# OpenSLAM-org/openslam_g2o

Hardware: AMD Instinct MI355X
Metric: linear-solve ms/iter (buildSystem + setLambda + solve + restoreDiagonal), 100k-pose BA (lower is better)
Workload: dtype f64; 1 GPU; synthetic BA (BASELINE.json configs[3]): 100000 poses / 1000000 landmarks / 5000000 observations, BlockSolver_6_3 semantics, Schur + multifrontal block Cholesky, lambda=10; poses=100000, landmarks=1000000, edges=5000000, parallelism=1 GPU, edge_data=estimates+measurements in HBM, errors/Jacobians evaluated inside buildSystem, information=identity, declared for the whole edge set (not read per edge)

## Files before the change

### openslam_g2o_amd/csrc/block_solver.hip

```cpp
#include "block_solver.h"

#include <algorithm>
#include <atomic>
#include <chrono>
#include <cmath>
#include <cstring>
#include <numeric>

namespace g2ohip {

namespace {

constexpr int kThreads = 256;
constexpr int kMaxBlocks = 1024;

template <int CTRL>
__device__ __forceinline__ double dpp_permute(double v) {
  const int lo = __double2loint(v), hi = __double2hiint(v);
  const int lo2 = __builtin_amdgcn_update_dpp(lo, lo, CTRL, 0xf, 0xf, true);
  const int hi2 = __builtin_amdgcn_update_dpp(hi, hi, CTRL, 0xf, 0xf, true);
  return __hiloint2double(hi2, lo2);
}
template <int G>
__device__ __forceinline__ double group_sum(double v) {
  if (G >= 2) v += dpp_permute<0xB1>(v);
  if (G >= 4) v += dpp_permute<0x4E>(v);
  if (G >= 8) v += dpp_permute<0x141>(v);
  if (G >= 16) v += dpp_permute<0x140>(v);
  return v;
}

typedef double dbl2_u __attribute__((ext_vector_type(2), aligned(8)));
template <int N>
__device__ __forceinline__ void load_vec(const double* __restrict__ p, double (&v)[N]) {
#pragma unroll
  for (int i = 0; i + 1 < N; i += 2) {
    const dbl2_u t = *reinterpret_cast<const dbl2_u*>(p + i);
    v[i] = t.x;
    v[i + 1] = t.y;
  }
  if (N & 1) v[N - 1] = p[N - 1];
}
template <int N>
__device__ __forceinline__ void store_vec(double* __restrict__ p, const double (&v)[N]) {
#pragma unroll
  for (int i = 0; i + 1 < N; i += 2) {
    dbl2_u t;
    t.x = v[i];
    t.y = v[i + 1];
    *reinterpret_cast<dbl2_u*>(p + i) = t;
  }
  if (N & 1) p[N - 1] = v[N - 1];
}
typedef double dbl2_a __attribute__((ext_vector_type(2), aligned(16)));
template <int N>
__device__ __forceinline__ void lds_block(const double* p, double (&v)[N]) {
  if (N % 2 == 0) {
#pragma unroll
    for (int i = 0; i < N; i += 2) {
      const dbl2_a t = *reinterpret_cast<const dbl2_a*>(p + i);
      v[i] = t.x;
      v[i + 1] = t.y;
    }
  } else {
#pragma unroll
    for (int i = 0; i < N; ++i) v[i] = p[i];
  }
}
__device__ __forceinline__ int xcd_swizzle(int b, int nblocks) {
  const int per = nblocks >> 3;
  return (b < (per << 3)) ? (b & 7) * per + (b >> 3) : b;
}

__device__ __forceinline__ double robust_weight(int kind, double delta, double e2) {
  const double dsqr = delta * delta;
  switch (kind) {
    case 1: return (e2 <= dsqr) ? 1.0 : delta / sqrt(e2);
    case 2: return 1.0 / sqrt(e2 / dsqr + 1.0);
    case 3: return 1.0 / (e2 / dsqr + 1.0);
    case 4: return (e2 <= dsqr) ? 1.0 : 0.0;
    case 5: {
      double sc = (2.0 * delta) / (delta + e2);
      if (sc >= 1.0) sc = 1.0;
      return sc * sc;
    }
    default: return 1.0;
  }
}
__device__ __forceinline__ double robust_rho(int kind, double delta, double e2) {
  const double dsqr = delta * delta;
  switch (kind) {
    case 1: return (e2 <= dsqr) ? e2 : 2.0 * sqrt(e2) * delta - dsqr;
    case 2: return 2.0 * dsqr * (sqrt(e2 / dsqr + 1.0) - 1.0);
    case 3: return dsqr * log(e2 / dsqr + 1.0);
    case 4: return (e2 <= dsqr) ? e2 : dsqr;
    case 5: {
      double sc = (2.0 * delta) / (delta + e2);
      if (sc >= 1.0) sc = 1.0;
      return sc * e2 * sc;
    }
    default: return e2;
  }
}

template <bool CLS>
__device__ __forceinline__ int ba_edge_class(int camword, const double* __restrict__ ctab, double& f, double& cx, double& cy, int& kind,
                                             double& delta) {
  if constexpr (CLS) {
    const double* t = ctab + 5 * (size_t)((unsigned)camword >> 24);
    f = t[0]; cx = t[1]; cy = t[2]; kind = (int)t[3]; delta = t[4];
    return camword & 0xffffff;
  } else {
    return camword;
  }
}

template <int D, int DV, int G>
__global__ void __launch_bounds__(kThreads) assemble_vertex_kernel(int nV, const int* __restrict__ vptr, const int* __restrict__ vent,
                                       const double* __restrict__ J0, const double* __restrict__ J1,
                                       const double* __restrict__ omega, const double* __restrict__ err, int kind, double delta,
                                       double* __restrict__ H, const int* __restrict__ diag_blk, double* __restrict__ b,
                                       int accumulate, const double* __restrict__ rk) {
  const int gt = blockIdx.x * blockDim.x + threadIdx.x;
  const int v = gt / G, g = gt % G;
  const bool active = v < nV;
  double Hacc[DV * DV];
  double bacc[DV];
#pragma unroll
  for (int i = 0; i < DV * DV; ++i) Hacc[i] = 0.0;
#pragma unroll
  for (int i = 0; i < DV; ++i) bacc[i] = 0.0;
  const int k0 = active ? vptr[v] : 0, k1 = active ? vptr[v + 1] : 0;
  for (int k = k0 + g; k < k1; k += G) {
    const int ent = vent[k];
    const size_t e = (size_t)(ent >> 1);
    const double* Jp = ((ent & 1) ? J1 : J0) + e * (D * DV);
    const double* Op = omega + e * (D * D);
    const double* rp = err + e * D;
    double J[D * DV], O[D * D], r[D], Or[D];
    load_vec<D * DV>(Jp, J);
    load_vec<D * D>(Op, O);
    load_vec<D>(rp, r);
    double e2 = 0.0;
#pragma unroll
    for (int i = 0; i < D; ++i) {
      double t = 0.0;
#pragma unroll
      for (int j = 0; j < D; ++j) t += O[i + D * j] * r[j];
      Or[i] = t;
      e2 += r[i] * t;
    }
    const double w = rk ? robust_weight((int)rk[2 * e], rk[2 * e + 1], e2) : robust_weight(kind, delta, e2);
#pragma unroll
    for (int c = 0; c < DV; ++c) {
      double t = 0.0;
#pragma unroll
      for (int i = 0; i < D; ++i) t += J[i + D * c] * Or[i];
      bacc[c] -= w * t;
    }
#pragma unroll
    for (int c = 0; c < DV; ++c) {
      double OJ[D];
#pragma unroll
      for (int i = 0; i < D; ++i) {
        double t = 0.0;
#pragma unroll
        for (int j = 0; j < D; ++j) t += O[i + D * j] * J[j + D * c];
        OJ[i] = w * t;
      }
#pragma unroll
      for (int a = 0; a < DV; ++a) {
        double t = 0.0;
#pragma unroll
        for (int i = 0; i < D; ++i) t += J[i + D * a] * OJ[i];
        Hacc[a + DV * c] += t;
      }
    }
  }
  if (G > 1) {
#pragma unroll
    for (int i = 0; i < DV * DV; ++i) Hacc[i] = group_sum<G>(Hacc[i]);
#pragma unroll
// ... 882 lines not shown

__device__ __forceinline__ void ba_lm_accumulate(const BaEdgeLin& L, double (&H)[9], double (&b)[3], double (&OA)[6]) {
  const double w = L.w;
  const double O00 = w * L.O[0], O10 = w * L.O[1], O01 = w * L.O[2], O11 = w * L.O[3];
#pragma unroll
  for (int c = 0; c < 3; ++c) {
    OA[0 + 2 * c] = O00 * L.A[0 + 2 * c] + O01 * L.A[1 + 2 * c];
    OA[1 + 2 * c] = O10 * L.A[0 + 2 * c] + O11 * L.A[1 + 2 * c];
  }
  const double Or0 = O00 * L.r[0] + O01 * L.r[1], Or1 = O10 * L.r[0] + O11 * L.r[1];
#pragma unroll
  for (int c = 0; c < 3; ++c) {
    b[c] -= L.A[0 + 2 * c] * Or0 + L.A[1 + 2 * c] * Or1;
#pragma unroll
    for (int a = 0; a < 3; ++a) H[a + 3 * c] += L.A[0 + 2 * a] * OA[0 + 2 * c] + L.A[1 + 2 * a] * OA[1 + 2 * c];
  }
}
__device__ __forceinline__ void ba_hpl_block(const BaEdgeLin& L, const double (&OA)[6], double (&blk)[18]) {
#pragma unroll
  for (int c = 0; c < 3; ++c)
#pragma unroll
    for (int a = 0; a < 6; ++a) blk[a + 6 * c] = L.B[0 + 2 * a] * OA[0 + 2 * c] + L.B[1 + 2 * a] * OA[1 + 2 * c];
}

#ifndef G2OHIP_ASMLM_OCC
#define G2OHIP_ASMLM_OCC 4
#endif
template <int G, bool CLS = false>
__global__ void __launch_bounds__(kThreads, G2OHIP_ASMLM_OCC) ba_assemble_landmarks_kernel(
    int nL, const int* __restrict__ vptr, const int* __restrict__ vent, const double* __restrict__ cams, const double* __restrict__ pts,
    const int* __restrict__ cam_lm, const int* __restrict__ pt_lm, const double* __restrict__ meas_lm, const double* __restrict__ omega_lm,
    const int* __restrict__ hpl_lm, double f, double cx, double cy, int kind, double delta, double* __restrict__ Hll,
    double* __restrict__ bl, double* __restrict__ Hpl, double* __restrict__ err, int ident, const int* __restrict__ pl_colptr,
    int write_hpl, const double* __restrict__ ctab) {
  __shared__ __attribute__((aligned(16))) double stage[kThreads / 64][64 * 18];
  const int gt = blockIdx.x * blockDim.x + threadIdx.x;
  const int lm = gt / G, g = gt % G;
  const bool active = lm < nL;
  const int wave = threadIdx.x / 64, lane = threadIdx.x % 64;
  const int lm_w0 = min((gt - lane) / G, nL), lm_w1 = min(lm_w0 + 64 / G, nL);
  const int q_base = pl_colptr[lm_w0], nslots = pl_colptr[lm_w1] - q_base;
  const bool staged = nslots <= 64;
  double H[9], b[3];
#pragma unroll
  for (int i = 0; i < 9; ++i) H[i] = 0.0;
  b[0] = b[1] = b[2] = 0.0;
  const int k0 = active ? vptr[lm] : 0, k1 = active ? vptr[lm + 1] : 0;
  for (int k = k0 + g; k < k1; k += G) {
    const int e = vent[k] >> 1;
    double T[12], X[3], z2[2], Op[4];
    const double* Xp = pts + (size_t)pt_lm[k] * 3;
    X[0] = Xp[0]; X[1] = Xp[1]; X[2] = Xp[2];
    load_vec<12>(cams + (size_t)ba_edge_class<CLS>(cam_lm[k], ctab, f, cx, cy, kind, delta) * 12, T);
    load_vec<2>(meas_lm + (size_t)k * 2, z2);
    if (ident) {
      Op[0] = Op[3] = 1.0;
      Op[1] = Op[2] = 0.0;
    } else {
      load_vec<4>(omega_lm + (size_t)k * 4, Op);
    }
    BaEdgeLin L;
    ba_edge_linearize(T, X, z2, Op, f, cx, cy, kind, delta, true, L);
    store_vec<2>(err + (size_t)e * 2, L.r);
    double OA[6];
    ba_lm_accumulate(L, H, b, OA);
    const int q = write_hpl ? hpl_lm[k] : -1;
    if (q >= 0) {
      double blk[18];
      ba_hpl_block(L, OA, blk);
      if (staged) store_vec<18>(&stage[wave][(q - q_base) * 18], blk);
      else store_vec<18>(Hpl + (size_t)q * 18, blk);
    }
  }
  if (staged && write_hpl) {
    __builtin_amdgcn_wave_barrier();
    const dbl2_u* src = reinterpret_cast<const dbl2_u*>(&stage[wave][0]);
    dbl2_u* dst = reinterpret_cast<dbl2_u*>(Hpl + (size_t)q_base * 18);
    for (int t = lane; t < nslots * 9; t += 64) dst[t] = src[t];
  }
  if (G > 1) {
#pragma unroll
    for (int i = 0; i < 9; ++i) H[i] = group_sum<G>(H[i]);
#pragma unroll
    for (int i = 0; i < 3; ++i) b[i] = group_sum<G>(b[i]);
  }
  if (!active) return;
#pragma unroll
  for (int i = 0; i < 9; ++i)
    if (G == 1 || (i % G) == g) Hll[(size_t)lm * 9 + i] = H[i];
#pragma unroll
  for (int i = 0; i < 3; ++i)
    if (G == 1 || (i % G) == g) bl[(size_t)lm * 3 + i] = b[i];
}

template <int G, bool FLL, bool CLS = false>
__global__ void __launch_bounds__(kThreads, G2OHIP_SCHUR_OCC) ba_schur_tile_kernel(
    const int* __restrict__ tile_lm0, const double* __restrict__ cams, const double* __restrict__ pts, const int* __restrict__ cam_q,
    const int* __restrict__ pt_q, const double* __restrict__ meas_q, const double* __restrict__ omega_q, double f, double cx, double cy,
    int kind, double delta, int ident, double* __restrict__ Dinv, double* bl, const int* __restrict__ td_diag,
    const int* __restrict__ td_ptr, const int* __restrict__ te_pack, const unsigned short* __restrict__ te_lm, double* __restrict__ Pd,
    double* __restrict__ Pr, double* Hll, const double* __restrict__ lam, const int4* __restrict__ ll_rec,
    const int4* __restrict__ tile_ll, const int* __restrict__ ll_edge, double* __restrict__ err, const int2* __restrict__ tile_q2,
    int store_hll, const unsigned short* __restrict__ slot_lm, const double* __restrict__ ctab) {
  extern __shared__ __attribute__((aligned(16))) double smem[];
  constexpr int PD = 6, LD = 3, PL = PD * LD;
  const int t = xcd_swizzle(blockIdx.x, gridDim.x);
  const int* tm = tile_lm0 + (size_t)t * 8;
  const int l0 = tm[0], l1 = tm[1], q0 = tm[2], nslots = tm[3], nlm = l1 - l0;
  const int td0 = tm[4], td1 = tm[5], e0 = tm[6], ne = tm[7];
  const int2 t2 = FLL ? make_int2(0, 0) : tile_q2[t];
  const int ntot = nslots + t2.y;
  double* Bs = smem;
  double* Ds = Bs + ((ntot * PL + 1) & ~1);
  double* bsm = Ds + ((nlm * LD * LD + 1) & ~1);
  double* Cs = bsm + ((nlm * LD + 1) & ~1);
  int* ep = reinterpret_cast<int*>(Cs + nlm * TileSplit<LD>::CP);
  int* dptr = ep + ne;
  int* ddiag = dptr + (td1 - td0 + 1);
  int* neg_flag = ddiag + (td1 - td0);
  unsigned short* el = reinterpret_cast<unsigned short*>(neg_flag + kThreads / 64);
  const int tid = threadIdx.x, NT = blockDim.x;
  if ((tid & 63) == 0) neg_flag[tid >> 6] = 0;
  const int slot_lm_first = FLL ? 0 : (int)slot_lm[q0 + min(tid, nslots - 1)];
  {
    const double* srcD = Hll + (size_t)l0 * LD * LD;
    const double* srcb = bl + (size_t)l0 * LD;
    const int nD = nlm * LD * LD, nb = nlm * LD, ndp = td1 - td0 + 1;
    constexpr int UD = 3, UE = 4;
    double vD[UD], vb;
    int vE[UE], vP, vG;
    unsigned short vL[UE];
    const int s0 = min(tid, nslots - 1);
    int cq = 0, pq = 0;
    if constexpr (!FLL) {
      cq = cam_q[q0 + s0];
      pq = pt_q[q0 + s0];
#pragma unroll
      for (int u = 0; u < UD; ++u) vD[u] = srcD[min(tid + u * NT, nD - 1)];
      vb = srcb[min(tid, nb - 1)];
    }
    auto request_lists = [&]() {
#pragma unroll
      for (int u = 0; u < UE; ++u) {
        const int i = min(tid + u * NT, ne - 1);
        vE[u] = te_pack[e0 + i];
        vL[u] = te_lm[e0 + i];
      }
      vP = td_ptr[td0 + min(tid, ndp - 1)];
      vG = td_diag[td0 + min(tid, max(ndp - 2, 0))];
    };
    request_lists();
    if constexpr (FLL) {
      const int4 tl = tile_ll[t];
      for (int sb = 0; sb < tl.y; sb += NT) {
        const int si = sb + tid;
        const size_t sg = (size_t)tl.x + min(si, tl.y - 1);
        int4 rc = ll_rec[sg];
        if (si >= tl.y) rc.x = (int)0x80000fffu;
        const int ent = rc.x;
        const int krel = ent & 0xfff, K = (ent >> 12) & 0xff, lmi = (ent >> 20) & 0x7ff;
        const bool has = krel != 0xfff, head = ent >= 0;
        const int pos = head ? 0 : lmi;
        double v[9];
        double Bk[12], OAk[6];
#pragma unroll
        for (int i = 0; i < 12; ++i) Bk[i] = 0.0;
#pragma unroll
        for (int i = 0; i < 6; ++i) OAk[i] = 0.0;
#pragma unroll
        for (int i = 0; i < 9; ++i) v[i] = 0.0;
        {
          const int ci = ba_edge_class<CLS>(rc.y, ctab, f, cx, cy, kind, delta), pi = rc.z, q = rc.w, e = ll_edge[sg];
          double T[12], X[3], z2[2], Op[4];
          const double* Xp = pts + (size_t)pi * 3;
          X[0] = Xp[0]; X[1] = Xp[1]; X[2] = Xp[2];
          load_vec<12>(cams + (size_t)ci * 12, T);
          load_vec<2>(meas_q + sg * 2, z2);
          if (ident) {
            Op[0] = Op[3] = 1.0;
            Op[1] = Op[2] = 0.0;
          } else {
            load_vec<4>(omega_q + sg * 4, Op);
          }
          if (has && !(store_hll & 8)) {
            BaEdgeLin L;
            ba_edge_linearize(T, X, z2, Op, f, cx, cy, kind, delta, true, L);
            if (err) store_vec<2>(err + (size_t)e * 2, L.r);
            double H[9], b[3], OA[6];
#pragma unroll
            for (int i = 0; i < 9; ++i) H[i] = 0.0;
            b[0] = b[1] = b[2] = 0.0;
            ba_lm_accumulate(L, H, b, OA);
            v[0] = H[0]; v[1] = H[1]; v[2] = H[2]; v[3] = H[4]; v[4] = H[5]; v[5] = H[8];
#pragma unroll
            for (int i = 0; i < 3; ++i) v[6 + i] = b[i];
            if (q >= 0) {
#pragma unroll
              for (int i = 0; i < 12; ++i) Bk[i] = L.B[i];
#pragma unroll
              for (int i = 0; i < 6; ++i) OAk[i] = OA[i];
            }
          }
        }
        for (int d = 1; __any(pos + d < K); d <<= 1) {
          const double take = pos + d < K ? 1.0 : 0.0;
          double o[9];
#pragma unroll
          for (int i = 0; i < 9; ++i) o[i] = __shfl_down(v[i], d);
#pragma unroll
          for (int i = 0; i < 9; ++i) v[i] = fma(o[i], take, v[i]);
        }
        double C[9];
#pragma unroll
        for (int i = 0; i < 9; ++i) C[i] = 0.0;
        if (head) {
          const int lm = l0 + lmi;
          double* bd = bl + (size_t)lm * 3;
          double Hf[9] = {v[0], v[1], v[2], v[1], v[3], v[4], v[2], v[4], v[5]};
          if (store_hll & 1) {
            double* hd = Hll + (size_t)lm * 9;
#pragma unroll
            for (int i = 0; i < 9; ++i) hd[i] = Hf[i];
          }
#pragma unroll
          for (int i = 0; i < 3; ++i) bd[i] = v[6 + i];
          double R[9], sg[3], u[3];
          const double lambda = lam[1];
          Hf[0] += lambda; Hf[4] += lambda; Hf[8] += lambda;
          small_inverse<3>(Hf, R);
          store_vec<9>(Dinv + (size_t)lm * 9, R);
          if (landmark_split<3>(R, v + 6, C, sg, u)) neg_flag[tid >> 6] = 1;
#pragma unroll
          for (int i = 0; i < 3; ++i) {
            Cs[lmi * TileSplit<3>::CP + 9 + i] = sg[i];
            bsm[lmi * 3 + i] = u[i];
          }
        }
        {
          const int src = (int)(threadIdx.x & 63) - pos;
          C[0] = __shfl(C[0], src); C[1] = __shfl(C[1], src); C[2] = __shfl(C[2], src);
          C[4] = __shfl(C[4], src); C[5] = __shfl(C[5], src); C[8] = __shfl(C[8], src);
          if (has && rc.w >= 0) {
            double OAC[6], V[18];
#pragma unroll
            for (int c = 0; c < 3; ++c)
#pragma unroll
              for (int r = 0; r < 2; ++r) {
                double t = OAk[r + 2 * c] * C[c + 3 * c];
#pragma unroll
                for (int k = c + 1; k < 3; ++k) t = fma(OAk[r + 2 * k], C[k + 3 * c], t);
                OAC[r + 2 * c] = t;
              }
#pragma unroll
            for (int c = 0; c < 3; ++c)
#pragma unroll
              for (int a = 0; a < 6; ++a)
                V[VSlot<PD, LD, (G >= 2 ? 2 : 1)>::off(a, c)] = Bk[0 + 2 * a] * OAC[0 + 2 * c] + Bk[1 + 2 * a] * OAC[1 + 2 * c];
            store_vec<18>(Bs + (rc.w - q0) * 18, V);
          }
        }
      }
    } else {
      for (int sb = 0; sb < ntot; sb += NT) {
        const int s_ = sb + tid;
        const int sc = min(s_, ntot - 1);
        const int qq = sc < nslots ? q0 + sc : t2.x + (sc - nslots);
        const bool pre = sb == 0 && s_ < nslots;
        const int c_ = ba_edge_class<CLS>(pre ? cq : cam_q[qq], ctab, f, cx, cy, kind, delta), p_ = pre ? pq : pt_q[qq];
        double T[12], X[3], z2[2], Op[4];
        load_vec<12>(cams + (size_t)c_ * 12, T);
        const double* Xp = pts + (size_t)p_ * 3;
        X[0] = Xp[0]; X[1] = Xp[1]; X[2] = Xp[2];
        load_vec<2>(meas_q + (size_t)qq * 2, z2);
        if (ident) {
          Op[0] = Op[3] = 1.0;
          Op[1] = Op[2] = 0.0;
        } else {
          load_vec<4>(omega_q + (size_t)qq * 4, Op);
        }
        BaEdgeLin L;
        ba_edge_linearize(T, X, z2, Op, f, cx, cy, kind, delta, true, L);
        const double w = L.w;
        const double O00 = w * L.O[0], O10 = w * L.O[1], O01 = w * L.O[2], O11 = w * L.O[3];
        double OA[6], blk[18];
#pragma unroll
        for (int c = 0; c < 3; ++c) {
          OA[0 + 2 * c] = O00 * L.A[0 + 2 * c] + O01 * L.A[1 + 2 * c];
          OA[1 + 2 * c] = O10 * L.A[0 + 2 * c] + O11 * L.A[1 + 2 * c];
        }
        ba_hpl_block(L, OA, blk);
        if (s_ < ntot) store_vec<18>(Bs + s_ * 18, blk);
      }
#pragma unroll
      for (int u = 0; u < UD; ++u) {
        const int i = tid + u * NT;
        if (i < nD) Ds[i] = vD[u];
      }
      if (tid < nb) bsm[tid] = vb;
    }
#pragma unroll
    for (int u = 0; u < UE; ++u) {
      const int i = tid + u * NT;
      if (i < ne) {
        ep[i] = vE[u];
        el[i] = vL[u];
      }
    }
    if (tid < ndp) dptr[tid] = vP;
    if (tid < ndp - 1) ddiag[tid] = vG;
    if constexpr (!FLL) {
      if (nD > UD * NT) stage_copy<4>(Ds + UD * NT, srcD + UD * NT, nD - UD * NT, tid, NT);
      if (nb > NT) stage_copy<2>(bsm + NT, srcb + NT, nb - NT, tid, NT);
    }
    if (ne > UE * NT) {
      stage_copy<4>(ep + UE * NT, te_pack + e0 + UE * NT, ne - UE * NT, tid, NT);
      stage_copy<4>(el + UE * NT, te_lm + e0 + UE * NT, ne - UE * NT, tid, NT);
    }
    if (ndp > NT) stage_copy<2>(dptr + NT, td_ptr + td0 + NT, ndp - NT, tid, NT);
    if (ndp - 1 > NT) stage_copy<2>(ddiag + NT, td_diag + td0 + NT, ndp - 1 - NT, tid, NT);
  }
  __syncthreads();
  if (!FLL) schur_tile_prepare<PD, LD, ((PD % 2 == 0 && G >= 2) ? 2 : 1)>(Bs, Ds, bsm, Cs, neg_flag, l0, nlm, ntot, slot_lm_first, slot_lm, q0, nslots, Dinv, Hll, lam, tid, NT);
  if (!(store_hll & 2)) schur_tile_dests<PD, LD, G>(Bs, Cs, bsm, tile_flag(neg_flag), ep, dptr, ddiag, el, td0, td1, e0, Pd, Pr, tid, NT);
}

template <int G, bool CLS = false>
__global__ void __launch_bounds__(kThreads) ba_back_substitute_kernel(
    int nL, const int* __restrict__ vptr, const double* __restrict__ cams, const double* __restrict__ pts,
    const int* __restrict__ cam_lm, const int* __restrict__ pt_lm, const double* __restrict__ meas_lm, const double* __restrict__ omega_lm,
    const int* __restrict__ row_lm, double f, double cx, double cy, int kind, double delta, int ident,
    const double* __restrict__ Dinv, const double* __restrict__ bl, const double* __restrict__ xp, double* __restrict__ xl,
    const double* __restrict__ ctab) {
  const int gt = blockIdx.x * blockDim.x + threadIdx.x;
  const int lm = gt / G, g = gt % G;
  const bool active = lm < nL;
  double c[3] = {0.0, 0.0, 0.0};
  const int k0 = active ? vptr[lm] : 0, k1 = active ? vptr[lm + 1] : 0;
  for (int k = k0 + g; k < k1; k += G) {
    const int row = row_lm[k];
    if (row < 0) continue;
    double T[12], X[3], z2[2], Op[4], xv[6];
    const double* Xp = pts + (size_t)pt_lm[k] * 3;
    X[0] = Xp[0]; X[1] = Xp[1]; X[2] = Xp[2];
    load_vec<12>(cams + (size_t)ba_edge_class<CLS>(cam_lm[k], ctab, f, cx, cy, kind, delta) * 12, T);
    load_vec<2>(meas_lm + (size_t)k * 2, z2);
    load_vec<6>(xp + (size_t)row * 6, xv);
    if (ident) {
      Op[0] = Op[3] = 1.0;
      Op[1] = Op[2] = 0.0;
    } else {
      load_vec<4>(omega_lm + (size_t)k * 4, Op);
    }
    BaEdgeLin L;
    ba_edge_linearize(T, X, z2, Op, f, cx, cy, kind, delta, true, L);
    double t0 = 0.0, t1 = 0.0;
#pragma unroll
    for (int a = 0; a < 6; ++a) {
      t0 += L.B[0 + 2 * a] * xv[a];
      t1 += L.B[1 + 2 * a] * xv[a];
    }
    const double w = L.w;
    const double u0 = w * (L.O[0] * t0 + L.O[2] * t1), u1 = w * (L.O[1] * t0 + L.O[3] * t1);
#pragma unroll
    for (int j = 0; j < 3; ++j) c[j] -= L.A[0 + 2 * j] * u0 + L.A[1 + 2 * j] * u1;
  }
  if (G > 1) {
#pragma unroll
    for (int j = 0; j < 3; ++j) c[j] = group_sum<G>(c[j]);
  }
  if (!active || g >= 3) return;
  double cl[3];
#pragma unroll
  for (int j = 0; j < 3; ++j) cl[j] = c[j] + bl[(size_t)lm * 3 + j];
  const double* D = Dinv + (size_t)lm * 9;
  if (G == 1) {
#pragma unroll
    for (int i = 0; i < 3; ++i) xl[(size_t)lm * 3 + i] = D[i] * cl[0] + D[i + 3] * cl[1] + D[i + 6] * cl[2];
  } else {
    xl[(size_t)lm * 3 + g] = D[g] * cl[0] + D[g + 3] * cl[1] + D[g + 6] * cl[2];
  }
}

template <bool CLS>
__global__ void __launch_bounds__(kThreads) ba_back_substitute_slots_kernel(
    const int* __restrict__ tile_lm0, const int4* __restrict__ tile_ll, const int4* __restrict__ ll_rec, const int* __restrict__ ll_row,
    const double* __restrict__ ll_meas, const double* __restrict__ ll_omega, const double* __restrict__ cams,
    const double* __restrict__ pts, double f, double cx, double cy, int kind, double delta, int ident, const double* __restrict__ Dinv,
    const double* __restrict__ bl, const double* __restrict__ xp, double* __restrict__ xl, const double* __restrict__ ctab) {
  const int t = blockIdx.x, tid = threadIdx.x, NT = blockDim.x;
  const int l0 = tile_lm0[(size_t)t * 8];
  const int4 tl = tile_ll[t];
  for (int sb = 0; sb < tl.y; sb += NT) {
    const int si = sb + tid;
    const size_t sg = (size_t)tl.x + min(si, tl.y - 1);
    int4 rc = ll_rec[sg];
    if (si >= tl.y) rc.x = (int)0x80000fffu;
    const int ent = rc.x;
    const int krel = ent & 0xfff, K = (ent >> 12) & 0xff, lmi = (ent >> 20) & 0x7ff;
    const bool head = ent >= 0;
    const int pos = head ? 0 : lmi;
    const int row = krel != 0xfff ? ll_row[sg] : -1;
    double c[3] = {0.0, 0.0, 0.0};
    {
      double T[12], X[3], z2[2], Op[4], xv[6];
      const double* Xp = pts + (size_t)rc.z * 3;
      X[0] = Xp[0]; X[1] = Xp[1]; X[2] = Xp[2];
      load_vec<12>(cams + (size_t)ba_edge_class<CLS>(rc.y, ctab, f, cx, cy, kind, delta) * 12, T);
      load_vec<2>(ll_meas + sg * 2, z2);
      load_vec<6>(xp + (size_t)max(row, 0) * 6, xv);
      if (ident) {
        Op[0] = Op[3] = 1.0;
        Op[1] = Op[2] = 0.0;
      } else {
        load_vec<4>(ll_omega + sg * 4, Op);
      }
      if (row >= 0) {
        BaEdgeLin L;
        ba_edge_linearize(T, X, z2, Op, f, cx, cy, kind, delta, true, L);
        double t0 = 0.0, t1 = 0.0;
#pragma unroll
        for (int a = 0; a < 6; ++a) {
          t0 += L.B[0 + 2 * a] * xv[a];
          t1 += L.B[1 + 2 * a] * xv[a];
        }
        const double w = L.w;
        const double u0 = w * (L.O[0] * t0 + L.O[2] * t1), u1 = w * (L.O[1] * t0 + L.O[3] * t1);
#pragma unroll
        for (int j = 0; j < 3; ++j) c[j] = -(L.A[0 + 2 * j] * u0 + L.A[1 + 2 * j] * u1);
      }
    }
    for (int d = 1; d < tl.w; d <<= 1) {
      const bool take = pos + d < K;
#pragma unroll
      for (int i = 0; i < 3; ++i) {
        const double o = __shfl_down(c[i], d);
        if (take) c[i] += o;
      }
    }
    if (head) {
      const int lm = l0 + lmi;
      double cl[3];
#pragma unroll
      for (int j = 0; j < 3; ++j) cl[j] = c[j] + bl[(size_t)lm * 3 + j];
      const double* D = Dinv + (size_t)lm * 9;
#pragma unroll
      for (int i = 0; i < 3; ++i) xl[(size_t)lm * 3 + i] = D[i] * cl[0] + D[i + 3] * cl[1] + D[i + 6] * cl[2];
    }
  }
}

#ifndef G2OHIP_ASMP_OCC
#define G2OHIP_ASMP_OCC 2
#endif
template <int G, bool CLS = false>
__global__ void __launch_bounds__(kThreads, G2OHIP_ASMP_OCC) ba_assemble_poses_kernel(
    int nP, const int* __restrict__ vptr, const double* __restrict__ cams, const double* __restrict__ pts,
    const int* __restrict__ cam_pm, const int* __restrict__ pt_pm, const double* __restrict__ meas_pm, const double* __restrict__ omega_pm,
    double f, double cx, double cy, int kind, double delta, double* __restrict__ Hpp, const int* __restrict__ diag_blk,
    double* __restrict__ bp, int accumulate, int ident, const int* __restrict__ act, const double* __restrict__ ctab) {
  const int gt = blockIdx.x * blockDim.x + threadIdx.x;
  const int vi_ = gt / G, g = gt % G;
  const bool active = vi_ < nP;
  const int v = (act && active) ? act[vi_] : vi_;
  double H[21], b[6];
#pragma unroll
  for (int i = 0; i < 21; ++i) H[i] = 0.0;
#pragma unroll
  for (int i = 0; i < 6; ++i) b[i] = 0.0;
  const int k0 = active ? vptr[v] : 0, k1 = active ? vptr[v + 1] : 0;
  double T[12];
  const int kf = k0 + g;
  if (kf < k1) load_vec<12>(cams + (size_t)(cam_pm[kf] & (CLS ? 0xffffff : -1)) * 12, T);
  int pt1 = kf < k1 ? pt_pm[kf] : 0, pt2 = kf + G < k1 ? pt_pm[kf + G] : 0;
  double Xn[3] = {0.0, 0.0, 0.0}, z2n[2] = {0.0, 0.0}, Opn[4] = {1.0, 0.0, 0.0, 1.0};
  if (kf < k1) {
    const double* Xp = pts + (size_t)pt1 * 3;
    Xn[0] = Xp[0]; Xn[1] = Xp[1]; Xn[2] = Xp[2];
    load_vec<2>(meas_pm + (size_t)kf * 2, z2n);
    if (!ident) load_vec<4>(omega_pm + (size_t)kf * 4, Opn);
  }
  for (int k = kf; k < k1; k += G) {
    double X[3], z2[2], Op[4];
    X[0] = Xn[0]; X[1] = Xn[1]; X[2] = Xn[2];
    z2[0] = z2n[0]; z2[1] = z2n[1];
#pragma unroll
    for (int i = 0; i < 4; ++i) Op[i] = Opn[i];
    {
      const int kn = k + G, kn2 = k + 2 * G;
      const int pt3 = kn2 < k1 ? pt_pm[kn2] : 0;
      if (kn < k1) {
        const double* Xp = pts + (size_t)pt2 * 3;
        Xn[0] = Xp[0]; Xn[1] = Xp[1]; Xn[2] = Xp[2];
        load_vec<2>(meas_pm + (size_t)kn * 2, z2n);
        if (!ident) load_vec<4>(omega_pm + (size_t)kn * 4, Opn);
      }
      pt2 = pt3;
    }
    if constexpr (CLS) (void)ba_edge_class<true>(cam_pm[k], ctab, f, cx, cy, kind, delta);
    BaEdgeLin L;
    ba_edge_linearize(T, X, z2, Op, f, cx, cy, kind, delta, false, L);
    const double w = L.w;
    const double O00 = w * L.O[0], O10 = w * L.O[1], O01 = w * L.O[2], O11 = w * L.O[3];
    const double Or0 = O00 * L.r[0] + O01 * L.r[1], Or1 = O10 * L.r[0] + O11 * L.r[1];
#pragma unroll
    for (int c = 0; c < 6; ++c) {
      const double OB0 = O00 * L.B[0 + 2 * c] + O01 * L.B[1 + 2 * c], OB1 = O10 * L.B[0 + 2 * c] + O11 * L.B[1 + 2 * c];
      b[c] -= L.B[0 + 2 * c] * Or0 + L.B[1 + 2 * c] * Or1;
#pragma unroll
      for (int a = 0; a <= c; ++a) H[c * (c + 1) / 2 + a] += L.B[0 + 2 * a] * OB0 + L.B[1 + 2 * a] * OB1;
    }
  }
  if (G > 1) {
#pragma unroll
    for (int i = 0; i < 21; ++i) H[i] = group_sum<G>(H[i]);
#pragma unroll
    for (int i = 0; i < 6; ++i) b[i] = group_sum<G>(b[i]);
  }
  if (!active) return;
  double* Hd = Hpp + (size_t)diag_blk[v] * 36;
  double* bd = bp + (size_t)v * 6;
#pragma unroll
  for (int i = 0; i < 36; ++i)
    if (G == 1 || (i % G) == g) {
      const int r_ = i % 6, c_ = i / 6, lo = r_ < c_ ? r_ : c_, hi = r_ < c_ ? c_ : r_;
      const double hv = H[hi * (hi + 1) / 2 + lo];
      Hd[i] = accumulate ? Hd[i] + hv : hv;
    }
#pragma unroll
  for (int i = 0; i < 6; ++i)
    if (G == 1 || (i % G) == g) bd[i] = accumulate ? bd[i] + b[i] : b[i];
}


__device__ __forceinline__ double pg_normalize_theta(double theta) {
  if (theta >= -M_PI && theta < M_PI) return theta;
  const double multiplier = floor(theta / (2 * M_PI));
  theta = theta - multiplier * 2 * M_PI;
  if (theta >= M_PI) theta -= 2 * M_PI;
  if (theta < -M_PI) theta += 2 * M_PI;
  return theta;
}
__device__ __forceinline__ void pg_se2_inverse(const double* a, double* r) {
  const double th = pg_normalize_theta(-a[2]), c = cos(th), s = sin(th);
  r[0] = c * (-a[0]) - s * (-a[1]);
  r[1] = s * (-a[0]) + c * (-a[1]);
  r[2] = th;
}
__device__ __forceinline__ void pg_se2_mul(const double* a, const double* b, double* r) {
  const double c = cos(a[2]), s = sin(a[2]);
  const double x = a[0] + c * b[0] - s * b[1], y = a[1] + s * b[0] + c * b[1];
  r[0] = x;
  r[1] = y;
  r[2] = pg_normalize_theta(a[2] + b[2]);
}
__global__ void __launch_bounds__(kThreads) pg_se2_linearize_kernel(int n, const double* __restrict__ poses, const int* __restrict__ vi,
                                                                  const int* __restrict__ vj, const double* __restrict__ meas,
                                                                  double* __restrict__ J0, double* __restrict__ J1,
                                                                  double* __restrict__ err, int jac) {
  const int k = blockIdx.x * blockDim.x + threadIdx.x;
  if (k >= n) return;
  const double* xi = poses + 3 * (size_t)vi[k];
  const double* xj = poses + 3 * (size_t)vj[k];
  double invm[3], invi[3], t1[3], delta[3];
  pg_se2_inverse(meas + 3 * (size_t)k, invm);
  pg_se2_inverse(xi, invi);
  pg_se2_mul(invi, xj, t1);
  pg_se2_mul(invm, t1, delta);
  err[3 * (size_t)k] = delta[0];
  err[3 * (size_t)k + 1] = delta[1];
  err[3 * (size_t)k + 2] = delta[2];
  if (!jac) return;
  const double thetai = xi[2], dtx = xj[0] - xi[0], dty = xj[1] - xi[1];
  const double si = sin(thetai), ci = cos(thetai);
  const double A[9] = {-ci, -si, -si * dtx + ci * dty, si, -ci, -ci * dtx - si * dty, 0, 0, -1};
  const double B[9] = {ci, si, 0, -si, ci, 0, 0, 0, 1};
  const double cz = cos(invm[2]), sz = sin(invm[2]);
  const double Z[9] = {cz, -sz, 0, sz, cz, 0, 0, 0, 1};
  double* o0 = J0 + 9 * (size_t)k;
  double* o1 = J1 + 9 * (size_t)k;
#pragma unroll
  for (int r = 0; r < 3; ++r)
#pragma unroll
    for (int c = 0; c < 3; ++c) {
      double a = 0, b = 0;
#pragma unroll
      for (int m = 0; m < 3; ++m) {
        a += Z[r * 3 + m] * A[m * 3 + c];
        b += Z[r * 3 + m] * B[m * 3 + c];
      }
// ... 2747 lines not shown
    rec[sidx] = r;
    edge[sidx] = ed;
    srow[sidx] = row;
    ms[2 * sidx] = m0;
    ms[2 * sidx + 1] = m1;
    if (os)
      for (int j = 0; j < 4; ++j) os[4 * sidx + j] = o[j];
  }
}

void BlockSolver::ba_set_edges_classes(int set, const int* cam_vertex, const int* point_vertex, const double* meas, const double* info,
                                       double f, double cx, double cy, int n_classes, const double* class_params, const int* edge_class) {
  invalidate_graphs();
  require_structure();
  if (set < 0 || set >= (int)sets_.size()) throw ArgFailure("bad edge set id");
  EdgeSet& es = *sets_[set];
  if (es.d != 2 || es.unary || es.dim0 != 3 || es.dim1 != 6 || p_ != 6 || l_ != 3)
    throw ArgFailure("ba_set_edges: the set must be EdgeProjectXYZ2UV-shaped (d=2, vertex0 = 3-dof point, vertex1 = 6-dof pose)");
  if (!cam_vertex || !point_vertex || !meas) throw ArgFailure("ba_set_edges: null array");
  G2OHIP_HIP_CHECK(hipSetDevice(device_));
  const size_t n = (size_t)es.n;
  const bool lapt = getenv("G2OHIP_SETUP_TIMING") != nullptr;
  auto lap_now = [] { return std::chrono::duration<double>(std::chrono::steady_clock::now().time_since_epoch()).count(); };
  double lap_t = lap_now();
  auto lap = [&](const char* what) {
    if (!lapt) return;
    const double t = lap_now();
    fprintf(stderr, "ba_set_edges: %-37s %.3f s\n", what, t - lap_t);
    lap_t = t;
  };
  if (n_classes < 1 || n_classes > 128) throw ArgFailure("ba_set_edges_classes: 1 to 128 edge classes");
  if (n_classes > 1 && (!class_params || !edge_class)) throw ArgFailure("ba_set_edges_classes: null class table");
  if (es.rk.p)
    throw StateFailure("ba_set_edges: the set carries per-edge robust kernels (set_robust_kernel_per_edge); on the BA front end they go through ba_set_edges_classes -- clear them first");
  std::vector<int> camc;
  if (n_classes > 1) {
    for (int c = 0; c < n_classes; ++c) {
      const double kd = class_params[5 * c + 3];
      if (!(kd == 0.0 || kd == 1.0 || kd == 2.0 || kd == 3.0 || kd == 4.0 || kd == 5.0)) throw ArgFailure("ba_set_edges_classes: robust kernel kind of a class must be 0..5");
      if (kd != 0.0 && !(class_params[5 * c + 4] > 0.0)) throw ArgFailure("ba_set_edges_classes: robust kernel delta of class " + std::to_string(c) + " must be positive");
    }
    camc.resize(n);
    for (size_t k = 0; k < n; ++k) {
      if (edge_class[k] < 0 || edge_class[k] >= n_classes) throw ArgFailure("ba_set_edges_classes: class of edge " + std::to_string(k) + " outside the table");
      if (cam_vertex[k] < 0 || cam_vertex[k] >= (1 << 24)) throw ArgFailure("ba_set_edges_classes: camera indices are limited to 2^24 with edge classes");
      camc[k] = cam_vertex[k] | (edge_class[k] << 24);
    }
  }
  ba_validate_edges(es, cam_vertex, point_vertex, n, ba_.cams.h_hidx.data(), ba_.cams.n, ba_.pts.h_hidx.data(), ba_.pts.n);
  std::vector<int> edge_hpl(n, -1);
  bool unique = es.first_lm && es.first_ol;
  {
    std::vector<char> seen(pl_row.size(), 0);
    for (size_t k = 0; k < n; ++k)
      if (es.v0[k] < 0) unique = false;
    host_parallel_for(n, [&](size_t b_, size_t e_) {
      for (size_t k = b_; k < e_; ++k) {
        const int a = es.v0[k], b = es.v1[k];
        if (a >= 0 && b >= 0) edge_hpl[k] = find_block(pl_colptr, pl_row, a - nP_, b);
      }
    });
    for (size_t k = 0; k < n; ++k) {
      const int q = edge_hpl[k];
      if (q < 0) continue;
      if (seen[q]) unique = false;
      seen[q] = 1;
    }
    if (n_classes > 1 && !unique)
      throw ArgFailure("ba_set_edges_classes: edge classes need the fused path (one observation per (pose, landmark) pair, no fixed landmark)");
  }
  lap("validation + Hpl block per edge");
  ba_.set = set;
  ba_.n_edges = es.n;
  ba_.f = f; ba_.cx = cx; ba_.cy = cy;
  ba_.stereo = false;
  ba_.baseline = 0;
  ba_.n_classes = n_classes;
  if (n_classes > 1) {
    ba_.h_ctab.assign(class_params, class_params + 5 * (size_t)n_classes);
    ba_.ctab.upload(ba_.h_ctab, st_);
    ba_.f = class_params[0]; ba_.cx = class_params[1]; ba_.cy = class_params[2];
    es.kernel_kind = (int)class_params[3];
    es.delta = class_params[4];
  } else {
    ba_.h_ctab.clear();
  }
  ba_.h_cam_v.assign(cam_vertex, cam_vertex + n);
  ba_.h_pt_v.assign(point_vertex, point_vertex + n);
  if (n_classes > 1) cam_vertex = camc.data();
  ba_.err_valid = ba_.jac_valid = false;
  chi2_valid_ = false;
  es.has_err = false;
  ba_.cam_v.upload(cam_vertex, n, st_);
  ba_.pt_v.upload(point_vertex, n, st_);
  ba_.meas.upload(meas, n * 2, st_);
  ba_.omega_identity = info == nullptr;
  if (!info) {
    es.own_omega.alloc(n * 4);
    if (n) hipLaunchKernelGGL(identity2_kernel, dim3(grid_for(n)), dim3(kThreads), 0, st_, n, es.own_omega.p);
  } else {
    es.own_omega.upload(info, n * 4, st_);
  }
  lap("uploads in edge order");
  const double* d_omega = ba_.omega_identity ? (const double*)nullptr : es.own_omega.p;
  auto zero_alloc = [&](auto& buf, size_t count) {
    buf.alloc(std::max<size_t>(count, 1));
    buf.zero(st_);
  };
  {
    ba_.fused_ok = unique;
    ba_.edge_hpl.upload(edge_hpl, st_);
    if (unique) {
      const size_t nq = std::max<size_t>(pl_row.size(), 1);
      zero_alloc(ba_.cam_q, nq);
      zero_alloc(ba_.pt_q, nq);
      zero_alloc(ba_.meas_q, nq * 2);
      if (d_omega) zero_alloc(ba_.omega_q, nq * 4);
      if (n)
        hipLaunchKernelGGL(ba_gather_blocks_kernel, dim3(grid_for(n)), dim3(kThreads), 0, st_, n, ba_.edge_hpl.p, ba_.cam_v.p, ba_.pt_v.p,
                           ba_.meas.p, d_omega, ba_.cam_q.p, ba_.pt_q.p, ba_.meas_q.p, d_omega ? ba_.omega_q.p : (double*)nullptr);
    }
  }
  lap("copies in Hpl block order");
  {
    const size_t nk = es.h_vp_ent.size(), nl = es.h_vl_ent.size();
    DevBuf<int> d_v1;
    d_v1.upload(es.v1, st_);
    ba_.meas_pm.alloc(std::max<size_t>(nk * 2, 1));
    ba_.pt_pm.alloc(std::max<size_t>(nk, 1));
    ba_.cam_pm.alloc(std::max<size_t>(nk, 1));
    if (d_omega) ba_.omega_pm.alloc(std::max<size_t>(nk * 4, 1));
    if (nk)
      hipLaunchKernelGGL(ba_gather_lists_kernel, dim3(grid_for(nk)), dim3(kThreads), 0, st_, nk, es.vp_ent.p, ba_.cam_v.p, ba_.pt_v.p, ba_.meas.p,
                         d_omega, (const int*)nullptr, (const int*)nullptr, ba_.cam_pm.p, ba_.pt_pm.p, ba_.meas_pm.p,
                         d_omega ? ba_.omega_pm.p : (double*)nullptr, (int*)nullptr, (int*)nullptr);
    ba_.meas_lm.alloc(std::max<size_t>(nl * 2, 1));
    ba_.cam_lm.alloc(std::max<size_t>(nl, 1));
    ba_.pt_lm.alloc(std::max<size_t>(nl, 1));
    ba_.hpl_lm.alloc(std::max<size_t>(nl, 1));
    ba_.row_lm.alloc(std::max<size_t>(nl, 1));
    if (d_omega) ba_.omega_lm.alloc(std::max<size_t>(nl * 4, 1));
    if (nl)
      hipLaunchKernelGGL(ba_gather_lists_kernel, dim3(grid_for(nl)), dim3(kThreads), 0, st_, nl, es.vl_ent.p, ba_.cam_v.p, ba_.pt_v.p, ba_.meas.p,
                         d_omega, ba_.edge_hpl.p, d_v1.p, ba_.cam_lm.p, ba_.pt_lm.p, ba_.meas_lm.p,
                         d_omega ? ba_.omega_lm.p : (double*)nullptr, ba_.hpl_lm.p, ba_.row_lm.p);
    G2OHIP_HIP_CHECK(hipGetLastError());
    lap("pose-major + landmark-major copies");
    ba_.ll_slots_ok = false;
    if (schur_ && n_tiles_ > 0 && tiles_cover_all_ && n_split_tiles_ == 0 && (int)tile_lm0_h_.size() == n_tiles_ + 1 &&
        (int)es.h_vl_ptr.size() == nL_ + 1) {
      constexpr int kIdleSlot = (int)0x80000fffu;
      std::vector<int4> tl((size_t)n_tiles_);
      std::vector<int> cnt((size_t)n_tiles_, 0);
      std::atomic<bool> okf(true);
      auto walk = [&](int t, int* out, int& kmax) {
        const int l0 = tile_lm0_h_[t], l1 = tile_lm0_h_[t + 1];
        const int kb = es.h_vl_ptr[l0];
        int used = 0, total = 0;
        kmax = 0;
        for (int lm = l0; lm < l1; ++lm) {
          const int K = es.h_vl_ptr[lm + 1] - es.h_vl_ptr[lm], lmi = lm - l0;
          if (K > 64 || lmi >= 0x7ff || es.h_vl_ptr[lm + 1] - kb >= 0xfff) return -1;
          const int need = std::max(K, 1);
          if (used + need > 64) {
            if (out)
              for (int i = used; i < 64; ++i) out[total + i - used] = kIdleSlot;
            total += 64 - used;
            used = 0;
          }
          if (out) {
            if (K == 0) out[total] = 0xfff | (lmi << 20);
            for (int j = 0; j < K; ++j)
              out[total + j] = (es.h_vl_ptr[lm] + j - kb) | (K << 12) | (j == 0 ? (lmi << 20) : (int)(0x80000000u | ((unsigned)j << 20)));
          }
          total += need;
          used = (used + need) & 63;
          kmax = std::max(kmax, K);
        }
        if (used) {
          if (out)
            for (int i = used; i < 64; ++i) out[total + i - used] = kIdleSlot;
          total += 64 - used;
        }
        return total;
      };
      host_parallel_for((size_t)n_tiles_, [&](size_t t0_, size_t t1_) {
        for (size_t t = t0_; t < t1_; ++t) {
          int kmax = 0;
          const int c = walk((int)t, nullptr, kmax);
          if (c < 0) okf.store(false);
          cnt[t] = std::max(c, 0);
        }
      }, 64);
      size_t ns = 0;
      for (int t = 0; t < n_tiles_; ++t) {
        tl[t].x = (int)ns;
        ns += (size_t)cnt[t];
      }
      if (okf.load() && ns < ((size_t)1 << 31)) {
        std::vector<int> slots(std::max<size_t>(ns, 1), kIdleSlot);
        host_parallel_for((size_t)n_tiles_, [&](size_t t0_, size_t t1_) {
          for (size_t t = t0_; t < t1_; ++t) {
            int kmax = 0;
            walk((int)t, slots.data() + tl[t].x, kmax);
            tl[t] = make_int4(tl[t].x, cnt[t], es.h_vl_ptr[tile_lm0_h_[t]], kmax);
          }
        }, 64);
        const size_t nsa = slots.size();
        DevBuf<int> d_slots;
        d_slots.upload(slots, st_);
        ba_.tile_ll.upload(tl, st_);
        ba_.ll_rec.alloc(nsa);
        ba_.ll_edge.alloc(nsa);
        ba_.ll_row.alloc(nsa);
        ba_.ll_meas.alloc(nsa * 2);
        if (d_omega) ba_.ll_omega.alloc(nsa * 4);
        if (ns == 0) {
          const int4 idle = make_int4(kIdleSlot, 0, 0, -1);
          const int none = -1;
          ba_.ll_rec.upload(&idle, 1, st_);
          ba_.ll_row.upload(&none, 1, st_);
          ba_.ll_edge.zero(st_);
          ba_.ll_meas.zero(st_);
        } else {
          hipLaunchKernelGGL(ba_gather_slots_kernel, dim3(n_tiles_), dim3(kThreads), 0, st_, ba_.tile_ll.p, d_slots.p, es.vl_ent.p, ba_.cam_lm.p,
                             ba_.pt_lm.p, ba_.hpl_lm.p, ba_.row_lm.p, ba_.meas_lm.p, d_omega ? ba_.omega_lm.p : (const double*)nullptr,
                             ba_.ll_rec.p, ba_.ll_edge.p, ba_.ll_row.p, ba_.ll_meas.p, d_omega ? ba_.ll_omega.p : (double*)nullptr);
        }
        G2OHIP_HIP_CHECK(hipGetLastError());
        G2OHIP_HIP_CHECK(hipStreamSynchronize(st_));
        ba_.ll_slots_ok = true;
      }
    }
    lap("lane slots of the tiles");
    G2OHIP_HIP_CHECK(hipStreamSynchronize(st_));
  }
  lap("pose-major / landmark-major uploads");
  if (!(ba_fused && ba_.fused_ok)) {
    es.own_J0.alloc(n * 6);
    es.own_J1.alloc(n * 12);
  }
  es.own_err.alloc(n * 2);
  es.J0 = es.own_J0.p; es.J1 = es.own_J1.p; es.omega = es.own_omega.p; es.err = es.own_err.p;
  es.has_data = false;
  prepare_ba_tile_kernels();
  G2OHIP_HIP_CHECK(hipStreamSynchronize(st_));
  lap("buffers, kernel attributes, sync");
}

void BlockSolver::ba_set_stereo_edges(int set, const int* cam_vertex, const int* point_vertex, const double* meas, const double* info,
                                      double f, double cx, double cy, double baseline) {
  invalidate_graphs();
  require_structure();
  if (set < 0 || set >= (int)sets_.size()) throw ArgFailure("bad edge set id");
  EdgeSet& es = *sets_[set];
  if (es.d != 3 || es.unary || es.dim0 != 3 || es.dim1 != 6 || p_ != 6 || l_ != 3)
    throw ArgFailure("ba_set_stereo_edges: the set must be EdgeProjectXYZ2UVU-shaped (d=3, vertex0 = 3-dof point, vertex1 = 6-dof pose)");
  if (!cam_vertex || !point_vertex || !meas) throw ArgFailure("ba_set_stereo_edges: null array");
  if (!std::isfinite(f) || !std::isfinite(cx) || !std::isfinite(cy) || !std::isfinite(baseline))
    throw ArgFailure("ba_set_stereo_edges: non-finite camera parameters");
  if (f == 0.0) throw ArgFailure("ba_set_stereo_edges: the focal length must not be zero");
  if (es.rk.p)
    throw StateFailure("ba_set_stereo_edges: the set carries per-edge robust kernels (set_robust_kernel_per_edge) -- clear them first and set them again on the bound set");
  G2OHIP_HIP_CHECK(hipSetDevice(device_));
  const size_t n = (size_t)es.n;
  ba_validate_edges(es, cam_vertex, point_vertex, n, ba_.cams.h_hidx.data(), ba_.cams.n, ba_.pts.h_hidx.data(), ba_.pts.n);
  ba_.set = set;
  ba_.n_edges = es.n;
  ba_.f = f; ba_.cx = cx; ba_.cy = cy;
  ba_.stereo = true;
  ba_.baseline = baseline;
  ba_.n_classes = 1;
  ba_.h_ctab.clear();
  ba_.ctab.release();
  ba_.h_cam_v.assign(cam_vertex, cam_vertex + n);
  ba_.h_pt_v.assign(point_vertex, point_vertex + n);
  ba_.err_valid = ba_.jac_valid = false;
  chi2_valid_ = false;
  ba_.sys_version = -1;
  ba_.fused_ok = false;
  ba_.ll_slots_ok = false;
  for (DevBuf<int>* b : {&ba_.edge_hpl, &ba_.pt_pm, &ba_.cam_pm, &ba_.cam_q, &ba_.pt_q, &ba_.cam_lm, &ba_.pt_lm, &ba_.hpl_lm, &ba_.row_lm,
                         &ba_.ll_edge, &ba_.ll_row})
    b->release();
  for (DevBuf<double>* b : {&ba_.meas_pm, &ba_.omega_pm, &ba_.meas_lm, &ba_.omega_lm, &ba_.meas_q, &ba_.omega_q, &ba_.ll_meas, &ba_.ll_omega})
    b->release();
  ba_.ll_rec.release();
  ba_.tile_ll.release();
  ba_.cam_v.upload(cam_vertex, n, st_);
  ba_.pt_v.upload(point_vertex, n, st_);
  ba_.meas.upload(meas, n * 3, st_);
  ba_.omega_identity = info == nullptr;
  if (!info) {
    es.own_omega.alloc(n * 9);
    if (n) hipLaunchKernelGGL(identity3_kernel, dim3(grid_for(n * 9)), dim3(kThreads), 0, st_, n, es.own_omega.p);
  } else {
    es.own_omega.upload(info, n * 9, st_);
  }
  es.own_J0.alloc(n * 9);
  es.own_J1.alloc(n * 18);
  es.own_err.alloc(n * 3);
  es.J0 = es.own_J0.p; es.J1 = es.own_J1.p; es.omega = es.own_omega.p; es.err = es.own_err.p;
  es.external = false;
  es.has_data = false;
  es.has_err = false;
  G2OHIP_HIP_CHECK(hipGetLastError());
  G2OHIP_HIP_CHECK(hipStreamSynchronize(st_));
}

bool BlockSolver::ba_recompute_ok() const {
  if (!schur_ || p_ != 6 || l_ != 3 || ba_.set < 0 || !ba_fused || !ba_.fused_ok || ba_.cams.n <= 0) return false;
  if (ba_.sys_version < 0 || ba_.sys_version != ba_.est_version) return false;
  const EdgeSet& bs = *sets_[ba_.set];
  if (bs.kernel_kind != ba_.sys_kind || bs.delta != ba_.sys_delta) return false;
  for (size_t i = 0; i < sets_.size(); ++i)
    if ((int)i != ba_.set && sets_[i]->n > 0 && sets_[i]->touches_lm) return false;
  return true;
}

void BlockSolver::ba_validate_edges(const EdgeSet& es, const int* cam_v, const int* pt_v, size_t n, const int* cam_hidx, int nc,
                                    const int* pt_hidx, int np) const {
  if (n == 0 || nc == 0) return;
  for (size_t k = 0; k < n; ++k) {
    const int c = cam_v[k], q = pt_v[k];
    if (c < 0 || c >= nc) throw ArgFailure("ba: camera index " + std::to_string(c) + " of edge " + std::to_string(k) + " outside the estimate table");
    if (q < 0 || q >= np) throw ArgFailure("ba: point index " + std::to_string(q) + " of edge " + std::to_string(k) + " outside the estimate table");
    const int hc = cam_hidx[c], hp = pt_hidx[q];
    if (hc >= nP_ || hp >= nL_) throw ArgFailure("ba: hessian index of an estimate outside the structure");
    const int v1 = hc < 0 ? -1 : hc, v0 = hp < 0 ? -1 : nP_ + hp;
    if (es.v1[k] != v1 || es.v0[k] != v0)
      throw ArgFailure("ba: edge " + std::to_string(k) + " connects vertices (" + std::to_string(es.v0[k]) + ", " + std::to_string(es.v1[k]) +
                       ") in the edge set but estimates with hessian indices (" + std::to_string(v0) + ", " + std::to_string(v1) + ")");
  }
}

void BlockSolver::pg_validate(const EdgeSet& es, const int* vi, const int* vj, size_t n, const int* hidx, int nv) const {
  if (n == 0 || nv == 0) return;
  for (size_t k = 0; k < n; ++k) {
    const int a = vi[k], b = vj[k];
    if (a < 0 || a >= nv || b < 0 || b >= nv) throw ArgFailure("pg: vertex index of edge " + std::to_string(k) + " outside the estimate table");
    const int ha = hidx[a], hb = hidx[b];
    if (ha >= nP_ || hb >= nP_) throw ArgFailure("pg: hessian index of an estimate outside the structure");
    if (es.v0[k] != (ha < 0 ? -1 : ha) || es.v1[k] != (hb < 0 ? -1 : hb))
      throw ArgFailure("pg: edge " + std::to_string(k) + ": the estimates' hessian indices differ from the edge set's");
  }
}

void BlockSolver::pg_validate_priors(const EdgeSet& es, const int* vq, size_t n, const int* hidx, int nv) const {
  for (size_t k = 0; k < n; ++k) {
    const int a = vq[k];
    if (a < 0) throw ArgFailure("pg: negative vertex index in prior edge " + std::to_string(k));
    if (nv > 0) {
      if (a >= nv) throw ArgFailure("pg: pose index of prior edge " + std::to_string(k) + " outside the estimate table");
      const int ha = hidx[a];
      if (ha >= nP_) throw ArgFailure("pg: hessian index of an estimate outside the structure");
      if (es.v0[k] != (ha < 0 ? -1 : ha))
        throw ArgFailure("pg: prior edge " + std::to_string(k) + ": the pose's hessian index differs from the edge set's");
    }
  }
}

// ... 686 lines not shown
```

Before: 1.135 ms/iter.

## Align landmark slot segments to 16-lane rows and reduce with DPP row shifts

After: 1.123 ms/iter, median of 6. -1.0%, faster.

```diff
diff --git a/openslam_g2o_amd/csrc/block_solver.hip b/openslam_g2o_amd/csrc/block_solver.hip
--- a/openslam_g2o_amd/csrc/block_solver.hip
+++ b/openslam_g2o_amd/csrc/block_solver.hip
@@ -28,6 +28,17 @@
   if (G >= 8) v += dpp_permute<0x141>(v);
   if (G >= 16) v += dpp_permute<0x140>(v);
   return v;
+}
+
+constexpr int kRowAlignedTile = 0x100;
+template <int D, int N>
+__device__ __forceinline__ void row_suffix_step(double (&v)[N], int pos, int K) {
+  const double take = pos + D < K ? 1.0 : 0.0;
+  double o[N];
+#pragma unroll
+  for (int i = 0; i < N; ++i) o[i] = dpp_permute<0x100 + D>(v[i]);
+#pragma unroll
+  for (int i = 0; i < N; ++i) v[i] = fma(o[i], take, v[i]);
 }
 
 typedef double dbl2_u __attribute__((ext_vector_type(2), aligned(8)));
@@ -1216,6 +1227,7 @@
     request_lists();
     if constexpr (FLL) {
       const int4 tl = tile_ll[t];
+      const bool rows = (tl.w & kRowAlignedTile) != 0;
       for (int sb = 0; sb < tl.y; sb += NT) {
         const int si = sb + tid;
         const size_t sg = (size_t)tl.x + min(si, tl.y - 1);
@@ -1266,13 +1278,26 @@
             }
           }
         }
-        for (int d = 1; __any(pos + d < K); d <<= 1) {
-          const double take = pos + d < K ? 1.0 : 0.0;
-          double o[9];
-#pragma unroll
-          for (int i = 0; i < 9; ++i) o[i] = __shfl_down(v[i], d);
-#pragma unroll
-          for (int i = 0; i < 9; ++i) v[i] = fma(o[i], take, v[i]);
+        if (rows) {
+          if (__any(pos + 1 < K)) {
+            row_suffix_step<1>(v, pos, K);
+            if (__any(pos + 2 < K)) {
+              row_suffix_step<2>(v, pos, K);
+              if (__any(pos + 4 < K)) {
+                row_suffix_step<4>(v, pos, K);
+                if (__any(pos + 8 < K)) row_suffix_step<8>(v, pos, K);
+              }
+            }
+          }
+        } else {
+          for (int d = 1; __any(pos + d < K); d <<= 1) {
+            const double take = pos + d < K ? 1.0 : 0.0;
+            double o[9];
+#pragma unroll
+            for (int i = 0; i < 9; ++i) o[i] = __shfl_down(v[i], d);
+#pragma unroll
+            for (int i = 0; i < 9; ++i) v[i] = fma(o[i], take, v[i]);
+          }
         }
         double C[9];
 #pragma unroll
@@ -1493,12 +1518,25 @@
         for (int j = 0; j < 3; ++j) c[j] = -(L.A[0 + 2 * j] * u0 + L.A[1 + 2 * j] * u1);
       }
     }
-    for (int d = 1; d < tl.w; d <<= 1) {
-      const bool take = pos + d < K;
-#pragma unroll
-      for (int i = 0; i < 3; ++i) {
-        const double o = __shfl_down(c[i], d);
-        if (take) c[i] += o;
+    if (tl.w & kRowAlignedTile) {
+      if (__any(pos + 1 < K)) {
+        row_suffix_step<1>(c, pos, K);
+        if (__any(pos + 2 < K)) {
+          row_suffix_step<2>(c, pos, K);
+          if (__any(pos + 4 < K)) {
+            row_suffix_step<4>(c, pos, K);
+            if (__any(pos + 8 < K)) row_suffix_step<8>(c, pos, K);
+          }
+        }
+      }
+    } else {
+      for (int d = 1; __any(pos + d < K); d <<= 1) {
+        const bool take = pos + d < K;
+#pragma unroll
+        for (int i = 0; i < 3; ++i) {
+          const double o = __shfl_down(c[i], d);
+          if (take) c[i] += o;
+        }
       }
     }
     if (head) {
@@ -4552,8 +4590,10 @@
       constexpr int kIdleSlot = (int)0x80000fffu;
       std::vector<int4> tl((size_t)n_tiles_);
       std::vector<int> cnt((size_t)n_tiles_, 0);
+      std::vector<char> rowal((size_t)n_tiles_, 0);
+      static const bool slot_rows = !getenv("G2OHIP_SLOT_ROWS") || atoi(getenv("G2OHIP_SLOT_ROWS")) != 0;
       std::atomic<bool> okf(true);
-      auto walk = [&](int t, int* out, int& kmax) {
+      auto walk = [&](int t, int* out, int& kmax, bool rows) {
         const int l0 = tile_lm0_h_[t], l1 = tile_lm0_h_[t + 1];
         const int kb = es.h_vl_ptr[l0];
         int used = 0, total = 0;
@@ -4562,6 +4602,14 @@
           const int K = es.h_vl_ptr[lm + 1] - es.h_vl_ptr[lm], lmi = lm - l0;
           if (K > 64 || lmi >= 0x7ff || es.h_vl_ptr[lm + 1] - kb >= 0xfff) return -1;
           const int need = std::max(K, 1);
+          if (rows && need > 16) return -1;
+          if (rows && (used & 15) + need > 16) {
+            const int pad = 16 - (used & 15);
+            if (out)
+              for (int i = 0; i < pad; ++i) out[total + i] = kIdleSlot;
+            total += pad;
+            used = (used + pad) & 63;
+          }
           if (used + need > 64) {
             if (out)
               for (int i = used; i < 64; ++i) out[total + i - used] = kIdleSlot;
@@ -4587,9 +4635,10 @@
       host_parallel_for((size_t)n_tiles_, [&](size_t t0_, size_t t1_) {
         for (size_t t = t0_; t < t1_; ++t) {
           int kmax = 0;
-          const int c = walk((int)t, nullptr, kmax);
+          const int c = walk((int)t, nullptr, kmax, false);
           if (c < 0) okf.store(false);
           cnt[t] = std::max(c, 0);
+          rowal[t] = slot_rows && c > 0 && walk((int)t, nullptr, kmax, true) == c;
         }
       }, 64);
       size_t ns = 0;
@@ -4602,11 +4651,21 @@
         host_parallel_for((size_t)n_tiles_, [&](size_t t0_, size_t t1_) {
           for (size_t t = t0_; t < t1_; ++t) {
             int kmax = 0;
-            walk((int)t, slots.data() + tl[t].x, kmax);
-            tl[t] = make_int4(tl[t].x, cnt[t], es.h_vl_ptr[tile_lm0_h_[t]], kmax);
+            walk((int)t, slots.data() + tl[t].x, kmax, rowal[t] != 0);
+            tl[t] = make_int4(tl[t].x, cnt[t], es.h_vl_ptr[tile_lm0_h_[t]], kmax | (rowal[t] ? kRowAlignedTile : 0));
           }
         }, 64);
         const size_t nsa = slots.size();
+        if (getenv("G2OHIP_PLAN_DUMP")) {
+          int nrow = 0, max_slots = 0, max_lm = 0;
+          for (int t = 0; t < n_tiles_; ++t) {
+            nrow += rowal[t] != 0;
+            max_slots = std::max(max_slots, cnt[t]);
+            max_lm = std::max(max_lm, tile_lm0_h_[t + 1] - tile_lm0_h_[t]);
+          }
+          fprintf(stderr, "lane slots: %zu for %zu observations, %d of %d tiles row-aligned, at most %d slots and %d landmarks in a tile\n", ns,
+                  es.h_vl_ent.size(), nrow, n_tiles_, max_slots, max_lm);
+        }
         DevBuf<int> d_slots;
         d_slots.upload(slots, st_);
         ba_.tile_ll.upload(tl, st_);
```
